# facebookresearch/robust_cvd

Hardware: NVIDIA H100
Metric: flow_residual_constraints_per_sec_per_gn_iteration (higher is better)
Workload: dtype f64

## Files before the change

### robust_cvd_b200/csrc/rcvd_api.cu

```cuda
#include <algorithm>
#include <chrono>
#include <cmath>
#include <cstdarg>
#include <cstdio>
#include <cstring>
#include <dlfcn.h>
#include <limits>
#include <string>
#include <vector>

#include <cub/device/device_segmented_sort.cuh>
#include "rcvd_eval.cuh"
#include "rcvd_linalg.cuh"
#include "rcvd_update.cuh"
#include "rcvd_plan.h"
#include "rcvd_host.h"

using namespace rcvd;

static thread_local std::string g_err = "";
int set_err(int code, const char* fmt, ...) {
  char buf[512]; va_list ap; va_start(ap, fmt); vsnprintf(buf, sizeof(buf), fmt, ap); va_end(ap);
  g_err = buf; return code;
}
// ... 293 lines not shown
    CK(cub::DeviceSegmentedSort::SortPairs(nullptr, tmp_bytes, d_k0, d_k1, d_i0, d_i1, (int)n, p->pairs.groups(), d_off, d_off + 1, p->stream));
    CK(cudaMallocAsync(&d_tmp, std::max<size_t>(tmp_bytes, 16), p->stream));
    CK(cub::DeviceSegmentedSort::SortPairs(d_tmp, tmp_bytes, d_k0, d_k1, d_i0, d_i1, (int)n, p->pairs.groups(), d_off, d_off + 1, p->stream));
    if ((rc = launch(p, k_gather_records, (unsigned)((n * 6 + 255) / 256), 256, 0, p->stream, false, p->pairs.dev.records, d_i1, n, d_sorted))) return rc;
    CK(cudaFreeAsync(d_tmp, p->stream));
    CK(cudaGetLastError());
    p->pairs.dev.records = d_sorted; p->records_sorted = true;
  }
  UP(p->d_in_range, frames_to_internal(uperm, p->in_range.data(), 1, 1, 1));
  UP(p->d_median, frames_to_internal(uperm, p->median.data(), 1, 1, 1));
  if (!p->adaptive.empty()) {
    const size_t G = p->adaptive.size() / N;
    UP(p->d_adaptive, frames_to_internal(uperm, p->adaptive.data(), G, G, G));
  }
  {
    std::vector<float> locs; const int gx = p->cfg.scale_grid_x, gy = p->cfg.scale_grid_y;
    for (int y = 0; y < gy; ++y) for (int x = 0; x < gx; ++x) {
      const float fx = -1.f + 2.f * x / (gx - 1);
      const float fy = -1.f + 2.f * y / (gy - 1);
      locs.push_back(fx); locs.push_back(fy);
    }
    p->nscale = (int)(locs.size() / 2);
    UP(p->d_scale_locs, locs);
  }
  p->first_frame = 0; p->last_frame = -1;
  { bool any = false; for (int f = 0; f < N; ++f) if (p->in_range[f]) { if (!any) { p->first_frame = f; any = true; } p->last_frame = f; } }
  p->part_reg = p->pairs.num_tiles;
  p->part_trip = p->part_reg + (reg_counts(p->cfg, L, N, p->nscale).total + 127) / 128;
  p->part_dp = p->part_trip + p->trips.num_tiles;
  p->npartial = p->part_dp + p->dpairs.num_tiles;
  return RCVD_OK;
}
#undef UP

static int allocate_storage(rcvd_problem* p) {
  const int N = p->N; const Layout& L = p->L; const int npad = L.npad, nLoff = p->plan.nLoff; const size_t bs = (size_t)npad * npad; int rc;
  const size_t Upad = (size_t)N * npad, U = (size_t)N * L.nf;
  DA(p->d_x, U); DA(p->d_xc, U); DA(p->d_xsave, U);
  DA(p->d_g, 2 * Upad + 8); p->d_diagH = p->d_g + Upad + 8;
  DA(p->d_S, Upad); DA(p->d_lmdiag, Upad); DA(p->d_D2, Upad); DA(p->d_gs, Upad); DA(p->d_rhs, Upad);
  DA(p->d_g2, Upad + 8); DA(p->d_delta, Upad);
  DA(p->d_ytmp, Upad); DA(p->d_y, Upad); DA(p->d_Sy, Upad); DA(p->d_Hy, Upad); DA(p->d_scal, SC_N); DA(p->d_active, Upad); DA(p->d_fail, 1);
  DA(p->d_potrf_progress, (size_t)N);
  DA(p->d_partial, (size_t)p->npartial);
  if (p->eval_only) { DA(p->d_H, 1); DA(p->d_Lb, 1); DA(p->d_T, 1); DA(p->d_invL, 1); DA(p->d_invT, 1); }
  else {
    DA(p->d_H, p->plan.hblocks.size() * bs); DA(p->d_Lb, (size_t)(N + nLoff) * bs); DA(p->d_T, (size_t)std::max(nLoff, 1) * bs);
    DA(p->d_invL, (size_t)N * bs); DA(p->d_invT, (size_t)N * npad * 16);
  }
#undef DA
  {
    bool encoded = false;
    typedef CUresult (*EncodeFn)(CUtensorMap*, CUtensorMapDataType, cuuint32_t, void*, const cuuint64_t*, const cuuint64_t*, const cuuint32_t*, const cuuint32_t*,
                                 CUtensorMapInterleave, CUtensorMapSwizzle, CUtensorMapL2promotion, CUtensorMapFloatOOBfill);
    void* fn = nullptr; cudaDriverEntryPointQueryResult qres;
    if (cudaGetDriverEntryPoint("cuTensorMapEncodeTiled", &fn, cudaEnableDefault, &qres) == cudaSuccess && fn && qres == cudaDriverEntryPointSuccess) {
      const cuuint64_t gdim[2] = {(cuuint64_t)npad, (cuuint64_t)std::max(nLoff, 1) * npad};
      const cuuint64_t gstr[1] = {(cuuint64_t)npad * sizeof(double)};
      const cuuint32_t box[2] = {16u, (cuuint32_t)p->plan.upd_rb};
      const cuuint32_t estr[2] = {1u, 1u};
      const CUresult r = ((EncodeFn)fn)(&p->tmapT, CU_TENSOR_MAP_DATA_TYPE_FLOAT64, 2, p->d_T, gdim, gstr, box, estr, CU_TENSOR_MAP_INTERLEAVE_NONE,
                                        CU_TENSOR_MAP_SWIZZLE_128B, CU_TENSOR_MAP_L2_PROMOTION_L2_128B, CU_TENSOR_MAP_FLOAT_OOB_FILL_NONE);
      encoded = (r == CUDA_SUCCESS);
    }
    cudaGetLastError();
    if (!encoded) return set_err(RCVD_ERR_CUDA, "cuTensorMapEncodeTiled unavailable or failed: the TMA update kernel cannot run");
    CK(cudaFuncSetAttribute(k_update_tma<1>, cudaFuncAttributeMaxDynamicSharedMemorySize, (int)upd_smem_bytes(p->plan.upd_rb, 1)));
    CK(cudaFuncSetAttribute(k_update_tma<2>, cudaFuncAttributeMaxDynamicSharedMemorySize, (int)upd_smem_bytes(p->plan.upd_rb, 2)));
  }
  CK(cudaMallocHost((void**)&p->h_scal, (SC_N + 2) * sizeof(double)));
  p->h_fail = (int*)(p->h_scal + SC_N);
  CK(cudaMemsetAsync(p->d_x, 0, U * sizeof(double), p->stream));
  CK(cudaMemsetAsync(p->d_lmdiag, 0, Upad * sizeof(double), p->stream));
  CK(cudaMemsetAsync(p->d_S, 0, Upad * sizeof(double), p->stream));
  CK(cudaMemsetAsync(p->d_active, 0, Upad, p->stream));
  if ((rc = enqueue_residuals<EvalMode::MarkActive>(p, p->d_x, nullptr))) return rc;
  if ((rc = launch(p, k_finalize_mask, (int)((Upad + 255) / 256), 256, 0, p->stream, false, p->cfg, L, p->d_active, N))) return rc;
  if (p->nranks > 1) {
    const int r = nccl::AllReduce(p->d_active, p->d_active, Upad, nccl::kUint8, nccl::kMax, p->comm, p->stream);
    if (r != 0) return set_err(RCVD_ERR_NCCL, "ncclAllReduce(active mask) failed");
  }
  FactorKernels& fk = p->fk = factor_kernels(npad);
  if (fk.trinv_bytes > kMaxDynSmem) return set_err(RCVD_ERR_INVALID, "frame block too large for the panel-inverse kernel (npad=%d)", npad);
  CK(cudaFuncSetAttribute(k_trinv, cudaFuncAttributeMaxDynamicSharedMemorySize, (int)fk.trinv_bytes));
  CK(cudaFuncSetAttribute(k_accumulate_fast, cudaFuncAttributeMaxDynamicSharedMemorySize, kFastSmem));
  CK(cudaFuncSetAttribute(k_accumulate_runs, cudaFuncAttributeMaxDynamicSharedMemorySize, kRunSmem));
  if (fk.trsm_ll) {
    CK(cudaFuncSetAttribute(k_trsm_ll<2>, cudaFuncAttributeMaxDynamicSharedMemorySize, (int)fk.trsm_ll2_bytes));
    CK(cudaFuncSetAttribute(k_trsm_ll<2, true>, cudaFuncAttributeMaxDynamicSharedMemorySize, (int)fk.trsm_ll2_bytes));
    CK(cudaOccupancyMaxActiveBlocksPerMultiprocessor(&fk.trsm2_ctas_per_sm, k_trsm_ll<2, true>, 128, fk.trsm_ll2_bytes));
  }
  if (fk.trsm_ll4) {
    CK(cudaFuncSetAttribute(k_trsm_ll<4>, cudaFuncAttributeMaxDynamicSharedMemorySize, (int)fk.trsm_ll4_bytes));
    CK(cudaFuncSetAttribute(k_trsm_ll<4, true>, cudaFuncAttributeMaxDynamicSharedMemorySize, (int)fk.trsm_ll4_bytes));
  }
  if (fk.potrf_smem) CK(cudaFuncSetAttribute(k_potrf_smem, cudaFuncAttributeMaxDynamicSharedMemorySize, (int)fk.potrf_bytes));
  return RCVD_OK;
}

static int build_structure(rcvd_problem* p) {
  if (p->nranks > 1 && !p->dpairs.frames.empty()) return set_err(RCVD_ERR_INVALID, "depth-normalisation pairs are not sharded: they need a single-GPU problem (nranks = 1)");
  free_all(p);
  CK(cudaSetDevice(p->device));
  std::vector<int32_t> graph = p->struct_pairs.empty() ? p->pairs.frames : p->struct_pairs;
  graph.insert(graph.end(), p->dpairs.frames.begin(), p->dpairs.frames.end());
  if (const char* e = make_factor_plan(p->plan, p->cfg, graph, p->trips.frames, p->order_slack, p->nranks, p->rank, p->dist_enabled, p->num_sms))
    return set_err(RCVD_ERR_INVALID, "%s", e);
  while (p->ev_side.size() < 2 * p->plan.levels.size()) { cudaEvent_t e; CK(cudaEventCreateWithFlags(&e, cudaEventDisableTiming)); p->ev_side.push_back(e); }
  int rc;
  if ((rc = upload_plan(p)) || (rc = set_up_problem_data(p)) || (rc = allocate_storage(p))) return rc;
  CK(cudaStreamSynchronize(p->stream));
  p->structure_ready = true;
  return RCVD_OK;
}

static int allreduce(rcvd_problem* p, double* buf, size_t count) {
  if (p->nranks <= 1) return RCVD_OK;
  const int r = nccl::AllReduce(buf, buf, count, nccl::kFloat64, nccl::kSum, p->comm, p->stream);
  if (r != 0) return set_err(RCVD_ERR_NCCL, "ncclAllReduce failed: %s", nccl::GetErrorString ? nccl::GetErrorString(r) : "?");
  return RCVD_OK;
}
struct Seg { size_t first, count; };
static int grouped(rcvd_problem* p, double* base, size_t unit, const std::vector<Seg>& segs, bool bcast) {
  int r = nccl::GroupStart();
  for (size_t i = 0; i < segs.size() && r == 0; ++i) {
    if (segs[i].count == 0) continue;
    const int root = (int)(i % (size_t)p->nranks);
    double* ptr = base + segs[i].first * unit;
    r = bcast ? nccl::Broadcast(ptr, ptr, segs[i].count * unit, nccl::kFloat64, root, p->comm, p->stream)
              : nccl::Reduce(ptr, ptr, segs[i].count * unit, nccl::kFloat64, nccl::kSum, root, p->comm, p->stream);
  }
  const int r2 = nccl::GroupEnd();
  if (r == 0) r = r2;
  if (r != 0) return set_err(RCVD_ERR_NCCL, "grouped NCCL %s failed: %s", bcast ? "broadcast" : "reduce", nccl::GetErrorString ? nccl::GetErrorString(r) : "?");
  return RCVD_OK;
}

struct FactorSolve {
  enum { P_LOAD = 0, P_POTRF, P_TRINV, P_TRSM, P_GEMM, P_SOLVE };
  rcvd_problem* p; const FactorPlan& pl; const FactorKernels& fk; const int N, npad, strips; cudaStream_t st, side, inv;
  int prof_level = 0;
  bool side_used = false, inv_used = false;
  int side_joined = -1;

  explicit FactorSolve(rcvd_problem* p_)
      : p(p_), pl(p_->plan), fk(p_->fk), N(p_->N), npad(p_->L.npad), strips((npad + kTrsmStrip - 1) / kTrsmStrip), st(p_->stream), side(p_->side_stream),
        inv(p_->inv_stream) {}

  void mark(int cls) {
    if (!p->prof) return;
    cudaEvent_t e; cudaEventCreate(&e); cudaEventRecord(e, st); p->prof->push_back({cls < 0 ? cls : (cls | (prof_level << 8)), e});
  }
  template <class... Params, class... Args>
  int launch(int path, void (*kernel)(Params...), dim3 grid, dim3 block, size_t smem, cudaStream_t s, bool pdl, Args... args) {
    if (int rc = ::launch(p, kernel, grid, block, smem, s, pdl, args...)) return rc;
    p->paths[path]++;
    return RCVD_OK;
  }
  int wait(cudaStream_t waiter, cudaStream_t from, cudaEvent_t e) {
    CK(cudaEventRecord(e, from)); CK(cudaStreamWaitEvent(waiter, e, 0));
    return RCVD_OK;
  }
  int join_all(int level) {
    if (side_used) { if (int rc = wait(st, side, p->ev_join)) return rc; side_joined = 2 * level - 1; }
    if (inv_used) { if (int rc = wait(st, inv, p->ev_inv_join)) return rc; inv_used = false; }
    return RCVD_OK;
  }

  bool trsm_deep(const Level& v) const { return strips * v.ntrsm <= p->num_sms && fk.trsm_ll4; }
  bool streamed(const Level& v) const {
    return fk.trsm_ll && v.nown > 0 && v.ntrsm > 0 && fk.potrf_smem && strips * v.ntrsm <= (trsm_deep(v) ? 1 : fk.trsm2_ctas_per_sm) * p->num_sms;
  }

  int factor_diagonal(const int* frames, int nfr, bool pdl) {
    if (fk.potrf_smem)
      return launch(LP_POTRF_SMEM, k_potrf_smem, dim3(nfr), dim3(kPotrfSmemThreads), fk.potrf_bytes, st, pdl, p->d_Lb, p->d_invT, frames, npad,
                    p->d_fail, p->d_potrf_progress);
    for (int jb = 0; jb < npad / 16; ++jb) {
      if (int rc = launch(LP_POTRF_PANEL, k_potrf_panel, dim3(nfr), dim3(kPotrfThreads), 0, st, false, p->d_Lb, p->d_invT, frames, npad, jb, p->d_fail)) return rc;
      const int m = npad - (jb + 1) * 16, n64 = (m + 63) / 64;
      if (m > 0) { if (int rc = launch(LP_OTHER, k_potrf_trail, dim3(n64 * (n64 + 1) / 2, nfr), dim3(128), 0, st, false, p->d_Lb, frames, npad, jb)) return rc; }
    }
    return RCVD_OK;
  }

  int trsm(const Level& lv, const int* frames, int nfr, bool chain) {
    const bool inv_stream = fk.trsm_ll && p->overlap;
    if (inv_stream) { if (int rc = wait(inv, st, p->ev_fork)) return rc; inv_used = true; }
    if (int rc = launch(LP_TRINV, k_trinv, dim3(npad / 16, nfr), dim3(256), fk.trinv_bytes, inv_stream ? inv : st, false,
                        p->d_Lb, p->d_invT, p->d_invL, frames, npad)) return rc;
    mark(P_TRINV);
    if (lv.ntrsm == 0) return RCVD_OK;
    int rc;
    if (fk.trsm_ll) {
      const bool deep = trsm_deep(lv);
      decltype(&k_trsm_ll<2>) kernel = deep ? (chain ? k_trsm_ll<4, true> : k_trsm_ll<4>) : (chain ? k_trsm_ll<2, true> : k_trsm_ll<2>);
      if (chain) p->paths[LP_TRSM_STREAMED]++;
      rc = launch(deep ? LP_TRSM_LL4 : LP_TRSM_LL2, kernel, dim3(strips, lv.ntrsm), dim3(128), deep ? fk.trsm_ll4_bytes : fk.trsm_ll2_bytes, st, chain,
                  p->d_T, p->d_Lb, p->d_invT, p->d_trsm_tasks + lv.trsm_off, npad, chain ? p->d_potrf_progress : nullptr);
    } else {
      const int tiles = (npad + 63) / 64;
      rc = launch(LP_TRSM_GEMM, k_gemm_nt, dim3(tiles, tiles, lv.ntrsm), dim3(128), 0, st, false, p->d_T, p->d_Lb, p->d_invL,
                  p->d_trsm_tasks + lv.trsm_off, npad);
    }
    if (rc) return rc;
    mark(P_TRSM);
    return RCVD_OK;
  }

  int update(cudaStream_t s, int off, int n) {
    if (n <= p->num_sms)
      return launch(LP_UPD_TMA2, k_update_tma<2>, dim3(n), dim3(UpdShape<2>::threads), upd_smem_bytes(pl.upd_rb, 2), s, false,
                    p->tmapT, p->d_Lb, p->d_upd_items + off, n, p->d_upd_pairs, npad, pl.upd_neff, pl.upd_rb, 0);
    int grid = std::min(n, 2 * p->num_sms);
    if (p->upd_ipc > 0) grid = std::max(grid, (n + p->upd_ipc - 1) / p->upd_ipc);
    if (grid < n) p->paths[LP_UPD_TMA1_MULTI]++;
    return launch(LP_UPD_TMA1, k_update_tma<1>, dim3(grid), dim3(UpdShape<1>::threads), upd_smem_bytes(pl.upd_rb, 1), s, false,
                  p->tmapT, p->d_Lb, p->d_upd_items + off, n, p->d_upd_pairs, npad, pl.upd_neff, pl.upd_rb, 0);
  }

  int updates(int li) {
    const Level& lv = pl.levels[li];
    const bool u2 = lv.nit2[0] + lv.nit2[1] > 0;
    const bool fork_late = li + 1 < (int)pl.levels.size() && streamed(pl.levels[li + 1]);
    if (p->overlap && u2 && !fork_late) { if (int rc = wait(side, st, p->ev_fork)) return rc; }
    if (p->overlap) {
      int s = -1;
      for (int q = side_joined + 1; q < 2 * li; ++q) { const Level& v = pl.levels[q / 2]; if (v.nit2[q % 2] > 0 && v.join[q % 2] <= li) s = q; }
      if (s >= 0) { CK(cudaStreamWaitEvent(st, p->ev_side[s], 0)); side_joined = s; }
    }
    if (lv.nit > 0) { if (int rc = update(st, lv.it_off, lv.nit)) return rc; mark(P_GEMM); }
    if (p->overlap && u2 && fork_late) { if (int rc = wait(side, st, p->ev_fork)) return rc; }
    for (int h = 0; h < 2; ++h) if (lv.nit2[h] > 0) {
      if (int rc = update(p->overlap ? side : st, lv.it2_off[h], lv.nit2[h])) return rc;
      mark(P_GEMM);
      if (p->overlap) { CK(cudaEventRecord(p->ev_side[2 * li + h], side)); side_used = true; }
    }
    return RCVD_OK;
  }

  int broadcast_level(int li) {
    std::vector<Seg> segs;
    for (int q = 0; q < p->nranks; ++q) segs.push_back({(size_t)pl.tseg[(li * p->nranks + q) * 2], (size_t)pl.tseg[(li * p->nranks + q) * 2 + 1]});
    return grouped(p, p->d_T, (size_t)npad * npad, segs, true);
  }
  int phase_boundary() {
    if (int rc = join_all(pl.LB)) return rc;
    const size_t bsz = (size_t)npad * npad;
    std::vector<Seg> invs, tr;
    for (int q = 0; q < p->nranks; ++q) invs.push_back({(size_t)pl.fa_off[q], (size_t)pl.fa_cnt[q]});
    for (int q = 0; q < p->nranks; ++q) tr.push_back({(size_t)pl.fb_off[q], (size_t)pl.fb_cnt[q]});
    for (int q = 0; q < p->nranks; ++q) tr.push_back({(size_t)N + (size_t)pl.bseg[2 * q], (size_t)pl.bseg[2 * q + 1]});
    if (int rc = grouped(p, p->d_invL, bsz, invs, true)) return rc;
    return grouped(p, p->d_Lb, bsz, tr, true);
  }

  int substitution() {
    CK(cudaMemcpyAsync(p->d_rhs, p->d_gs, (size_t)N * npad * sizeof(double), cudaMemcpyDeviceToDevice, st));
    const int LS = pl.sub_first_level;
    int rc;
    for (int l = 0; l < LS; ++l) {
      const Level& lv = pl.levels[l];
      if ((rc = launch(LP_SUB_LEVEL, k_fwd_diag, dim3((npad + 7) / 8, lv.nframes), dim3(256), 0, st, false, p->d_invL, p->d_rhs, p->d_ytmp,
                       p->d_lvl_frames + lv.frame_off, npad))) return rc;
      if (lv.nfwd > 0 && (rc = launch(LP_SUB_LEVEL, k_fwd_update, dim3((npad + 7) / 8, lv.nfwd), dim3(256), 0, st, false, p->d_T, p->d_ytmp, p->d_rhs,
                                      p->d_fwd_tasks + lv.fwd_off, npad))) return rc;
    }
    if (LS < (int)pl.levels.size() && !pl.sub_tasks.empty()) {
      CK(cudaMemsetAsync(p->d_sub_counters, 0, ((size_t)4 * N + 4) * sizeof(int), st));
      SubCounters cn; cn.ticket = p->d_sub_counters; cn.fin = p->d_sub_counters + 4; cn.fdone = cn.fin + N; cn.bin = cn.fdone + N; cn.bdone = cn.bin + N;
      cn.fin_need = p->d_sub_need; cn.bin_need = p->d_sub_need + N;
      const int ntasks = (int)pl.sub_tasks.size();
// ... 979 lines not shown
```

### robust_cvd_b200/csrc/rcvd_linalg.cuh

```cuda
#pragma once
#include "rcvd_device.cuh"
#include "rcvd_ptx.cuh"

namespace rcvd {

constexpr int kPotrfThreads = 256;

__global__ void __launch_bounds__(kPotrfThreads) k_potrf_panel(double* __restrict__ Lb, double* __restrict__ invT,
                                                                const int* __restrict__ frames, int npad, int jb, int* __restrict__ fail) {
  __shared__ double D[16][17];
  __shared__ double Di[16][17];
  const int frame = frames[blockIdx.x];
  double* A = Lb + (size_t)frame * npad * npad;
  double* iT = invT + (size_t)frame * npad * 16;
  const int tid = threadIdx.x;
  const int j0 = jb * 16;
  {
    const int r = tid >> 4, cc = tid & 15;
    D[r][cc] = (cc <= r) ? A[(size_t)(j0 + r) * npad + j0 + cc] : 0.0;
  }
  __syncthreads();
  if (tid < 32) {
    const int i = tid;
    for (int j = 0; j < 16; ++j) {
// ... 188 lines not shown
  POTRF_PHASE(1);
  for (int jb = 0; jb < nt; ++jb) {
    const double* D = tiles + (size_t)(jb * (jb + 1) / 2 + jb) * kTileSz;
    const double* pv = pinv + jb * 16;
    const int rows = (nt - jb - 1) * 16;
    int prow = -1;
    const int nwork = nw - 1, widx = warp - 1;
    if (warp == 0) { if (lane < 16 && rows > 0) prow = lane; } else if (widx * 32 + lane < rows - 16) prow = 16 + widx * 32 + lane;
    if (warp != 0) {
      if (jb > 0) publish(jb - 1);
      named_bar_sync<2, kPotrfSmemThreads>();
    }
    if (prow >= 0) {
      const int ti = jb + 1 + (prow >> 4), r = prow & 15;
      double* Tt = tiles + (size_t)(ti * (ti + 1) / 2 + jb) * kTileSz;
      double a[16];
#pragma unroll
      for (int q = 0; q < 16; q += 2) { const double2 v = *reinterpret_cast<const double2*>(&Tt[swz(r, q)]); a[q] = v.x; a[q + 1] = v.y; }
#pragma unroll
      for (int q = 0; q < 16; q += 2) {
        const double2 pq = *reinterpret_cast<const double2*>(&pv[q]);
        const double2 dq = *reinterpret_cast<const double2*>(&D[swz(q + 1, q)]);
        a[q] *= pq.x;
        a[q + 1] = (a[q + 1] - a[q] * dq.x) * pq.y;
#pragma unroll
        for (int c = 0; c < 16; ++c) if (c > q + 1) { const double2 l = *reinterpret_cast<const double2*>(&D[swz(c, q)]); a[c] -= a[q] * l.x; a[c] -= a[q + 1] * l.y; }
      }
#pragma unroll
      for (int q = 0; q < 16; q += 2) *reinterpret_cast<double2*>(&Tt[swz(r, q)]) = make_double2(a[q], a[q + 1]);
    } else if (warp == nw - 1 && lane < 16) {
      const int cidx = lane;
      double xcol[16];
#pragma unroll
      for (int r = 0; r < 16; ++r) xcol[r] = (r == cidx) ? 1.0 : 0.0;
#pragma unroll
      for (int q = 0; q < 16; q += 2) {
        const double2 pq = *reinterpret_cast<const double2*>(&pv[q]);
        const double2 dq = *reinterpret_cast<const double2*>(&D[swz(q + 1, q)]);
        xcol[q] *= pq.x;
        xcol[q + 1] = (xcol[q + 1] - xcol[q] * dq.x) * pq.y;
#pragma unroll
        for (int r = 0; r < 16; ++r) if (r > q + 1) { const double2 l = *reinterpret_cast<const double2*>(&D[swz(r, q)]); xcol[r] -= l.x * xcol[q]; xcol[r] -= l.y * xcol[q + 1]; }
      }
#pragma unroll
      for (int r = 0; r < 16; ++r) iT[(size_t)jb * 256 + r * 16 + cidx] = xcol[r];
    }
    POTRF_PHASE(2);
    if (warp != 0) named_bar_sync<3, kPotrfSmemThreads - 32>();
    POTRF_PHASE(3);
    const int m = nt - jb - 1, ntr = m * (m + 1) / 2;
    auto upd_tile = [&](int gi, int gj) -> double* {
      const double* Xi = tiles + (size_t)(gi * (gi + 1) / 2 + jb) * kTileSz;
      const double* Xj = tiles + (size_t)(gj * (gj + 1) / 2 + jb) * kTileSz;
      double* Ct = tiles + (size_t)(gi * (gi + 1) / 2 + gj) * kTileSz;
      double acc[2][2][2] = {{{0.0, 0.0}, {0.0, 0.0}}, {{0.0, 0.0}, {0.0, 0.0}}};
      tile_mma_nt(Xi, Xj, acc, g, t);
#pragma unroll
      for (int i = 0; i < 2; ++i)
#pragma unroll
        for (int j = 0; j < 2; ++j) {
          double2* ptr = reinterpret_cast<double2*>(&Ct[swz(i * 8 + g, j * 8 + 2 * t)]);
          double2 v = *ptr; v.x -= acc[i][j][0]; v.y -= acc[i][j][1]; *ptr = v;
        }
      return Ct;
    };
    if (warp == 0) {
      double* Ct = nullptr;
      if (ntr > 0) { __syncwarp(); Ct = upd_tile(jb + 1, jb + 1); }
      __threadfence_block();
      named_bar_arrive<2, kPotrfSmemThreads>();
      POTRF_PHASE(4);
      if (ntr > 0) { __syncwarp(); warp_chol16_blocked(Ct, pinv + (jb + 1) * 16, lane, fail); }
      POTRF_PHASE(5);
    } else {
      for (int tl = 1 + widx; tl < ntr; tl += nwork) { const int2 tij = tri_index(tl); upd_tile(jb + 1 + tij.x, jb + 1 + tij.y); }
    }
    POTRF_PHASE(6);
    __syncthreads();
    POTRF_PHASE(7);
  }
  if (warp != 0) publish(nt - 1);
}

__global__ void __launch_bounds__(256) k_trinv(const double* __restrict__ Lb, const double* __restrict__ invT, double* __restrict__ invL,
                                                const int* __restrict__ frames, int npad) {
  extern __shared__ double Z[];
  __shared__ double W[16][17];
  const int frame = frames[blockIdx.y];
  const int j = blockIdx.x;
  const int nt = npad / 16;
  double* Lrow_s = Z + (size_t)nt * 256;
  const int ldp = npad + 1;
  const double* A = Lb + (size_t)frame * npad * npad;
  const double* iT = invT + (size_t)frame * npad * 16;
  double* out = invL + (size_t)frame * npad * npad;
  const int tid = threadIdx.x, r = tid >> 4, c = tid & 15;
  for (int i = 0; i < j; ++i) out[(size_t)(i * 16 + r) * npad + j * 16 + c] = 0.0;
  Z[(size_t)j * 256 + tid] = iT[(size_t)j * 256 + tid];
  out[(size_t)(j * 16 + r) * npad + j * 16 + c] = Z[(size_t)j * 256 + tid];
  __syncthreads();
  for (int i = j + 1; i < nt; ++i) {
    const int kw = (i - j) * 16;
    for (int e = tid; e < 16 * kw; e += 256) { const int rr = e / kw, kk = e % kw; Lrow_s[rr * ldp + kk] = A[(size_t)(i * 16 + rr) * npad + j * 16 + kk]; }
    __syncthreads();
    double s0 = 0.0, s1 = 0.0, s2 = 0.0, s3 = 0.0;
    const double* lr = Lrow_s + r * ldp;
    const double* zp = Z + (size_t)j * 256 + c;
    for (int kk = 0; kk < kw; kk += 4) {
      s0 += lr[kk] * zp[(size_t)kk * 16]; s1 += lr[kk + 1] * zp[(size_t)(kk + 1) * 16];
      s2 += lr[kk + 2] * zp[(size_t)(kk + 2) * 16]; s3 += lr[kk + 3] * zp[(size_t)(kk + 3) * 16];
    }
    W[r][c] = (s0 + s1) + (s2 + s3);
    __syncthreads();
    double zv = 0.0;
    const double* ti = iT + (size_t)i * 256;
#pragma unroll
    for (int q = 0; q < 16; ++q) zv -= ti[r * 16 + q] * W[q][c];
    Z[(size_t)i * 256 + tid] = zv;
    out[(size_t)(i * 16 + r) * npad + j * 16 + c] = zv;
    __syncthreads();
  }
}

struct TrsmTask { int dst; int src; int kframe; };

constexpr int kGemmLd = 20;

template <int NI, int NJ>
__device__ __forceinline__ void gemm_stage(const double* __restrict__ as, const double* __restrict__ bsm, double (&acc)[4][4][2], int wm, int wn, int g, int t) {
#pragma unroll
  for (int k4 = 0; k4 < 4; ++k4) {
    double af[NI > 0 ? NI : 1], bf[NJ > 0 ? NJ : 1];
#pragma unroll
    for (int i = 0; i < NI; ++i) af[i] = as[(wm + i * 8 + g) * kGemmLd + k4 * 4 + t];
#pragma unroll
    for (int j = 0; j < NJ; ++j) bf[j] = bsm[(wn + j * 8 + g) * kGemmLd + k4 * 4 + t];
#pragma unroll
    for (int i = 0; i < NI; ++i)
#pragma unroll
      for (int j = 0; j < NJ; ++j) dmma_8x8x4(acc[i][j][0], acc[i][j][1], af[i], bf[j]);
  }
}

__global__ void __launch_bounds__(128, 4) k_gemm_nt(double* __restrict__ T, const double* __restrict__ Lb, const double* __restrict__ invL,
                                                  const TrsmTask* __restrict__ tasks, int npad) {
  __shared__ __align__(16) double As[2][64 * kGemmLd];
  __shared__ __align__(16) double Bs[2][64 * kGemmLd];
  const TrsmTask task = tasks[blockIdx.z];
  const int m0 = blockIdx.y * 64, n0 = blockIdx.x * 64;
  const size_t bs = (size_t)npad * npad;
  const int tid = threadIdx.x, warp = tid >> 5, lane = tid & 31;
  const int wm = (warp >> 1) * 32, wn = (warp & 1) * 32;
  const int g = lane >> 2, t = lane & 3;
  const int kchunks = min(npad, n0 + 64) / 16;
  const int ni = min(4, max(0, (npad - (m0 + wm)) / 8)), nj = min(4, max(0, (npad - (n0 + wn)) / 8));
  double acc[4][4][2];
#pragma unroll
  for (int i = 0; i < 4; ++i)
#pragma unroll
    for (int j = 0; j < 4; ++j) { acc[i][j][0] = 0.0; acc[i][j][1] = 0.0; }

  auto load_stage = [&](int st, int kk) {
    const double* Ag = Lb + (size_t)task.src * bs + kk * 16;
    const double* Bg = invL + (size_t)task.kframe * bs + kk * 16;
#pragma unroll
    for (int q = 0; q < 4; ++q) {
      const int cidx = tid + q * 128;
      const int row = cidx >> 3, kc = (cidx & 7) * 2;
      const bool va = (m0 + row) < npad, vb = (n0 + row) < npad;
      cp_async16(&As[st][row * kGemmLd + kc], Ag + (size_t)(va ? m0 + row : 0) * npad + kc, va);
      cp_async16(&Bs[st][row * kGemmLd + kc], Bg + (size_t)(vb ? n0 + row : 0) * npad + kc, vb);
    }
    cp_async_commit();
  };

  load_stage(0, 0);
  for (int kk = 0; kk < kchunks; ++kk) {
    const int st = kk & 1;
    if (kk + 1 < kchunks) { load_stage(st ^ 1, kk + 1); cp_async_wait<1>(); } else { cp_async_wait<0>(); }
    __syncthreads();
    const double* as = As[st]; const double* bsm = Bs[st];
    if (ni == 4 && nj == 4) gemm_stage<4, 4>(as, bsm, acc, wm, wn, g, t);
    else if (ni == 4 && nj == 2) gemm_stage<4, 2>(as, bsm, acc, wm, wn, g, t);
    else if (ni == 2 && nj == 4) gemm_stage<2, 4>(as, bsm, acc, wm, wn, g, t);
    else if (ni == 2 && nj == 2) gemm_stage<2, 2>(as, bsm, acc, wm, wn, g, t);
    __syncthreads();
  }
  double* C = T + (size_t)task.dst * bs;
#pragma unroll
  for (int i = 0; i < 4; ++i) {
    const int row = m0 + wm + i * 8 + g;
    if (row >= npad) continue;
#pragma unroll
    for (int j = 0; j < 4; ++j) {
      const int col = n0 + wn + j * 8 + 2 * t;
      if (col >= npad) continue;
      *reinterpret_cast<double2*>(C + (size_t)row * npad + col) = make_double2(acc[i][j][0], acc[i][j][1]);
    }
  }
}

__global__ void __launch_bounds__(128, 4) k_potrf_trail(double* __restrict__ Lb, const int* __restrict__ frames, int npad, int jb) {
  __shared__ __align__(16) double Ps[2][64 * kGemmLd];
  const int frame = frames[blockIdx.y];
  double* A = Lb + (size_t)frame * npad * npad;
  const int j0 = jb * 16, j1 = j0 + 16;
// ... 92 lines not shown
        __syncthreads();
        ready = s_ready;
      }
      for (; staged < min(ready, jt + kTrsmAhead); ++staged) stage(staged);
      cp_async_wait_upto3(staged - 1 - jt);
    } else {
      cp_async_wait<kTrsmAhead - 1>();
    }
    __syncthreads();
    const double* ls = Ls + (size_t)(jt % kTrsmAhead) * 16 * ld; const double* dsm = Ds + (jt % kTrsmAhead) * 320;
    double acc[NI][2][2];
#pragma unroll
    for (int i = 0; i < NI; ++i) { acc[i][0][0] = acc[i][0][1] = acc[i][1][0] = acc[i][1][1] = 0.0; }
    {
      double af[2][4][NI], bf[2][4][2];
      auto frag = [&](int kt, int buf) {
#pragma unroll
        for (int q = 0; q < 4; ++q) {
#pragma unroll
          for (int i = 0; i < NI; ++i) af[buf][q][i] = Xs[(size_t)(wr + i * 8 + g) * ld + kt * 16 + q * 4 + t];
#pragma unroll
          for (int j = 0; j < 2; ++j) bf[buf][q][j] = ls[(size_t)(j * 8 + g) * ld + kt * 16 + q * 4 + t];
        }
      };
      if (jt > 0) frag(0, 0);
      for (int kt = 0; kt < jt; kt += 2) {
        if (kt + 1 < jt) frag(kt + 1, 1);
#pragma unroll
        for (int q = 0; q < 4; ++q)
#pragma unroll
          for (int i = 0; i < NI; ++i)
#pragma unroll
            for (int j = 0; j < 2; ++j) dmma_8x8x4(acc[i][j][0], acc[i][j][1], af[0][q][i], bf[0][q][j]);
        if (kt + 1 < jt) {
          if (kt + 2 < jt) frag(kt + 2, 0);
#pragma unroll
          for (int q = 0; q < 4; ++q)
#pragma unroll
            for (int i = 0; i < NI; ++i)
#pragma unroll
              for (int j = 0; j < 2; ++j) dmma_8x8x4(acc[i][j][0], acc[i][j][1], af[1][q][i], bf[1][q][j]);
        }
      }
    }
#pragma unroll
    for (int i = 0; i < NI; ++i)
#pragma unroll
      for (int j = 0; j < 2; ++j) {
        double2* ptr = reinterpret_cast<double2*>(&Xs[(size_t)(wr + i * 8 + g) * ld + jt * 16 + j * 8 + 2 * t]);
        double2 v = *ptr; v.x -= acc[i][j][0]; v.y -= acc[i][j][1]; *ptr = v;
      }
    __syncwarp();
    double out[NI][2][2];
#pragma unroll
    for (int i = 0; i < NI; ++i) { out[i][0][0] = out[i][0][1] = out[i][1][0] = out[i][1][1] = 0.0; }
#pragma unroll
    for (int k4 = 0; k4 < 4; ++k4) {
      double af[NI], bf[2];
#pragma unroll
      for (int i = 0; i < NI; ++i) af[i] = Xs[(size_t)(wr + i * 8 + g) * ld + jt * 16 + k4 * 4 + t];
#pragma unroll
      for (int j = 0; j < 2; ++j) bf[j] = dsm[(j * 8 + g) * 20 + k4 * 4 + t];
#pragma unroll
      for (int i = 0; i < NI; ++i)
#pragma unroll
        for (int j = 0; j < 2; ++j) dmma_8x8x4(out[i][j][0], out[i][j][1], af[i], bf[j]);
    }
    __syncwarp();
#pragma unroll
    for (int i = 0; i < NI; ++i)
#pragma unroll
      for (int j = 0; j < 2; ++j) {
        const int r = wr + i * 8 + g, cidx = jt * 16 + j * 8 + 2 * t;
        const double2 v = make_double2(out[i][j][0], out[i][j][1]);
        *reinterpret_cast<double2*>(&Xs[(size_t)r * ld + cidx]) = v;
        if (r < rows) *reinterpret_cast<double2*>(&X[(size_t)(m0 + r) * npad + cidx]) = v;
      }
    __syncthreads();
    if constexpr (!kStreamed) stage(jt + kTrsmAhead);
  }
  if constexpr (kStreamed) griddep_wait();
}


__global__ void __launch_bounds__(256) k_fwd_diag(const double* __restrict__ invL, const double* __restrict__ rhs, double* __restrict__ y,
                                                   const int* __restrict__ frames, int npad) {
  const int frame = frames[blockIdx.y];
  const int row = blockIdx.x * 8 + (threadIdx.x >> 5);
  const int lane = threadIdx.x & 31;
  if (row >= npad) return;
  const double* M = invL + (size_t)frame * npad * npad + (size_t)row * npad;
  const double* b = rhs + (size_t)frame * npad;
  double s = 0.0;
  for (int q = lane; q <= row; q += 32) s += M[q] * b[q];
  s = warp_sum(s);
  if (lane == 0) y[(size_t)frame * npad + row] = s;
}
struct SolveTask { int blk; int r; int k; };
__global__ void __launch_bounds__(256) k_fwd_update(const double* __restrict__ T, const double* __restrict__ y, double* __restrict__ rhs,
                                                     const SolveTask* __restrict__ tasks, int npad) {
  const SolveTask tk = tasks[blockIdx.y];
  const int row = blockIdx.x * 8 + (threadIdx.x >> 5);
  const int lane = threadIdx.x & 31;
  if (row >= npad) return;
  const double* M = T + (size_t)tk.blk * npad * npad + (size_t)row * npad;
  const double* v = y + (size_t)tk.k * npad;
  double s = 0.0;
  for (int q = lane; q < npad; q += 32) s += M[q] * v[q];
  s = warp_sum(s);
  if (lane == 0) red_add(rhs + (size_t)tk.r * npad + row, -s);
}
__global__ void __launch_bounds__(256) k_bwd_update(const double* __restrict__ T, const double* __restrict__ x, double* __restrict__ y,
                                                     const SolveTask* __restrict__ tasks, int npad) {
  __shared__ double red[8][33];
  const SolveTask tk = tasks[blockIdx.y];
  const int cl = threadIdx.x & 31, rg = threadIdx.x >> 5;
  const int j = blockIdx.x * 32 + cl;
  double acc = 0.0;
  if (j < npad) {
    const double* M = T + (size_t)tk.blk * npad * npad + j;
    const double* xr = x + (size_t)tk.r * npad;
    for (int i = rg; i < npad; i += 8) acc += M[(size_t)i * npad] * xr[i];
  }
  red[rg][cl] = acc;
  __syncthreads();
  if (rg == 0 && j < npad) {
    double s = 0.0;
#pragma unroll
    for (int q = 0; q < 8; ++q) s += red[q][cl];
    if (s != 0.0) red_add(y + (size_t)tk.k * npad + j, -s);
  }
}
__global__ void __launch_bounds__(256) k_bwd_diag(const double* __restrict__ invL, const double* __restrict__ y, double* __restrict__ x,
                                                   const int* __restrict__ frames, int npad) {
  __shared__ double red[8][33];
  const int frame = frames[blockIdx.y];
  const int cl = threadIdx.x & 31, rg = threadIdx.x >> 5;
  const int j = blockIdx.x * 32 + cl;
  double acc = 0.0;
  if (j < npad) {
    const double* M = invL + (size_t)frame * npad * npad + j;
    const double* v = y + (size_t)frame * npad;
    const int i0 = j - (j % 8) + rg;
    for (int i = (i0 < j ? i0 + 8 : i0); i < npad; i += 8) acc += M[(size_t)i * npad] * v[i];
  }
  red[rg][cl] = acc;
  __syncthreads();
  if (rg == 0 && j < npad) {
    double s = 0.0;
#pragma unroll
    for (int q = 0; q < 8; ++q) s += red[q][cl];
    x[(size_t)frame * npad + j] = s;
  }
}

constexpr int kSubChunk = 64;
constexpr int kSubThreads = 256;
struct SubTask { int type; int blk; int r; int k; int chunk; };
struct SubCounters { int* ticket; int* fin; int* fdone; int* bin; int* bdone; const int* fin_need; const int* bin_need; };

__device__ __forceinline__ void sub_wait(const int* c, int need) { while (ld_acquire_gpu(c) < need) __nanosleep(20); }

__device__ __forceinline__ double2 ldcg2(const double* p) { return __ldcg(reinterpret_cast<const double2*>(p)); }

__global__ void __launch_bounds__(kSubThreads) k_substitution(const double* __restrict__ invL, const double* __restrict__ T, double* rhs, double* y, double* x,
                                                              const SubTask* __restrict__ tasks, int ntasks, SubCounters cn, int npad) {
// ... 10 lines not shown
    const SubTask tk = tasks[ti];
    const int c0 = tk.chunk * kSubChunk, c1 = min(npad, c0 + kSubChunk);
    const double* vin = tk.type == 0 ? rhs + (size_t)tk.k * npad : (tk.type == 2 ? x + (size_t)tk.r * npad : y + (size_t)tk.k * npad);
    const double* M = (tk.type == 0 || tk.type == 3) ? invL + (size_t)tk.k * bs : T + (size_t)tk.blk * bs;
    auto dep_wait = [&]() {
      if (tid == 0) {
        if (tk.type == 0) sub_wait(cn.fin + tk.k, cn.fin_need[tk.k]);
        else if (tk.type == 1) sub_wait(cn.fdone + tk.k, nchunks);
        else if (tk.type == 2) sub_wait(cn.bdone + tk.r, nchunks);
        else { sub_wait(cn.fdone + tk.k, nchunks); sub_wait(cn.bin + tk.k, cn.bin_need[tk.k]); }
      }
      __syncthreads();
    };
    if (tk.type <= 1) {
      constexpr int RW = kSubChunk / (kSubThreads / 32);
      const int r0 = c0 + warp * RW;
      double acc[RW];
#pragma unroll
      for (int i = 0; i < RW; ++i) acc[i] = 0.0;
      for (int qb = 0; qb < npad; qb += 256) {
        double2 m[4][RW];
#pragma unroll
        for (int qi = 0; qi < 4; ++qi) {
          const int q = qb + qi * 64 + 2 * lane;
#pragma unroll
          for (int i = 0; i < RW; ++i) {
            const int row = r0 + i;
            const int len = tk.type == 0 ? row + 1 : npad;
            m[qi][i] = (row < c1 && q < len) ? *reinterpret_cast<const double2*>(M + (size_t)row * npad + q) : make_double2(0.0, 0.0);
            if (q + 1 >= len) m[qi][i].y = 0.0;
          }
        }
        if (qb == 0) dep_wait();
        double2 v[4];
#pragma unroll
        for (int qi = 0; qi < 4; ++qi) { const int q = qb + qi * 64 + 2 * lane; v[qi] = q < npad ? ldcg2(vin + q) : make_double2(0.0, 0.0); }
#pragma unroll
        for (int qi = 0; qi < 4; ++qi)
#pragma unroll
          for (int i = 0; i < RW; ++i) acc[i] += m[qi][i].x * v[qi].x + m[qi][i].y * v[qi].y;
      }
#pragma unroll
      for (int i = 0; i < RW; ++i) {
        const double sum = warp_sum(acc[i]);
        const int row = r0 + i;
        if (lane == 0 && row < c1) { if (tk.type == 0) y[(size_t)tk.k * npad + row] = sum; else red_add(rhs + (size_t)tk.r * npad + row, -sum); }
      }
    } else {
      const int cl = tid & 31, rg = tid >> 5, j = c0 + 2 * cl;
      double ax = 0.0, ay = 0.0;
      const int ifirst = tk.type == 3 ? j + ((rg - j) & 7) : rg;
      for (int ib = ifirst; ib < npad || ib == ifirst; ib += 256) {
        double2 m[32];
#pragma unroll
        for (int u = 0; u < 32; ++u) { const int i = ib + 8 * u; m[u] = (i < npad && j < c1) ? *reinterpret_cast<const double2*>(M + (size_t)i * npad + j) : make_double2(0.0, 0.0); }
        if (ib == ifirst) dep_wait();
        double vi[32];
#pragma unroll
        for (int u = 0; u < 32; ++u) { const int i = ib + 8 * u; vi[u] = i < npad ? __ldcg(vin + i) : 0.0; }
#pragma unroll
        for (int u = 0; u < 32; ++u) { const int i = ib + 8 * u; ax += m[u].x * vi[u]; if (tk.type != 3 || i > j) ay += m[u].y * vi[u]; }
      }
      red[rg * (kSubChunk + 2) + 2 * cl] = ax; red[rg * (kSubChunk + 2) + 2 * cl + 1] = ay;
      __syncthreads();
      if (tid < kSubChunk && c0 + tid < c1) {
        double sum = 0.0;
#pragma unroll
        for (int q = 0; q < 8; ++q) sum += red[q * (kSubChunk + 2) + tid];
        if (tk.type == 3) x[(size_t)tk.k * npad + c0 + tid] = sum; else red_add(y + (size_t)tk.k * npad + c0 + tid, -sum);
      }
    }
    __syncthreads();
    if (tid == 0) red_release_add(tk.type == 0 ? cn.fdone + tk.k : (tk.type == 1 ? cn.fin + tk.r : (tk.type == 2 ? cn.bin + tk.k : cn.bdone + tk.k)), 1);
  }
}

struct FactorKernels {
  bool potrf_smem, trsm_ll, trsm_ll4;
  size_t potrf_bytes, trsm_ll2_bytes, trsm_ll4_bytes, trinv_bytes, substitution_bytes;
  int trsm2_ctas_per_sm;
};
inline FactorKernels factor_kernels(int npad) {
  const size_t potrf = potrf_smem_bytes(npad), ll2 = trsm_ll_smem_bytes(npad, 2), ll4 = trsm_ll_smem_bytes(npad, 4);
  const size_t trinv = (size_t)(npad * 16 + 16 * (npad + 1)) * sizeof(double);
  const size_t sub = (size_t)8 * (kSubChunk + 2) * sizeof(double);
  return {potrf <= kMaxDynSmem, ll2 <= kMaxDynSmem, ll4 <= kMaxDynSmem, potrf, ll2, ll4, trinv, sub, 0};
}

struct HBlock { int lblk; int r; int c; };
__global__ void __launch_bounds__(256) k_load_factor(const double* __restrict__ H, double* __restrict__ Lb, const HBlock* __restrict__ lb,
                                                      const double* __restrict__ S, const double* __restrict__ D2, int npad, int nf, int neff,
                                                      const int* __restrict__ blist, int nload, int nfill) {
  const size_t bs = (size_t)npad * npad;
  if ((int)blockIdx.y >= nload) {
    const int ph = npad - neff, per = ph * (npad + neff);
    const long q = ((long)(blockIdx.y - nload) * gridDim.x + blockIdx.x) * 256 + threadIdx.x;
    if (per == 0 || q >= (long)nfill * per) return;
    const int f = (int)(q / per), e = (int)(q % per), r = e - ph * npad;
    const int i = r < 0 ? neff + e / npad : r / ph, j = r < 0 ? e % npad : neff + r % ph;
    Lb[(size_t)blist[nload + f] * bs + (size_t)i * npad + j] = 0.0;
    return;
  }
  const int bid = blist[blockIdx.y];
  const HBlock b = lb[bid];
  const int e = blockIdx.x * 256 + threadIdx.x;
  if (e >= npad * npad) return;
  const int i = e / npad, j = e % npad;
  double v = 0.0;
  if (b.r == b.c) {
    if (j > i) v = 0.0;
    else if (i >= nf) v = (i == j) ? 1.0 : 0.0;
    else {
      v = H[(size_t)b.lblk * bs + e] * S[(size_t)b.r * npad + i] * S[(size_t)b.c * npad + j];
      if (i == j) v += D2[(size_t)b.r * npad + i];
    }
  } else if (i < nf && j < nf) {
    v = H[(size_t)b.lblk * bs + e] * S[(size_t)b.r * npad + i] * S[(size_t)b.c * npad + j];
  }
  Lb[(size_t)bid * bs + e] = v;
}
__host__ __device__ inline int load_factor_pad_rows(int npad, int neff, int nfill) {
  const long per = (long)(npad - neff) * (npad + neff), row = (long)((npad * npad + 255) / 256) * 256;
  return (int)(((long)nfill * per + row - 1) / row);
}

__global__ void __launch_bounds__(256) k_spmv_sym(const double* __restrict__ H, const HBlock* __restrict__ hb, const double* __restrict__ v,
                                                   double* __restrict__ out, int npad, const int* __restrict__ blist) {
  const int bid = blist ? blist[blockIdx.y] : blockIdx.y;
  const HBlock b = hb[bid];
  const int row = blockIdx.x * 8 + (threadIdx.x >> 5);
  const int lane = threadIdx.x & 31;
  if (row >= npad) return;
  const double* M = H + (size_t)bid * npad * npad + (size_t)row * npad;
  const double* vc = v + (size_t)b.c * npad;
  const double vr = v[(size_t)b.r * npad + row];
  double s = 0.0;
  if (b.r == b.c) {
    for (int q = lane; q <= row; q += 32) {
      const double m = M[q];
      s += m * vc[q];
      if (q < row && m != 0.0) red_add(out + (size_t)b.c * npad + q, m * vr);
    }
  } else {
    for (int q = lane; q < npad; q += 32) {
      const double m = M[q];
      s += m * vc[q];
      if (m != 0.0 && vr != 0.0) red_add(out + (size_t)b.c * npad + q, m * vr);
    }
  }
  s = warp_sum(s);
  if (lane == 0 && s != 0.0) red_add(out + (size_t)b.r * npad + row, s);
}

}
```

Before: 84.82 million.

## Rewrite triangular inverse kernel as strip-based DMMA solve with cp.async staging

Replaces the per-column-block scalar triangular inverse with a strip-parallel kernel that computes inverse rows using FP64 tensor-core MMA (dmma_16x8x4). L panels and diagonal inverses are staged into shared memory with cp.async double-buffering when shared memory permits, and the kernel falls back to direct global loads otherwise. The aim is to cut the scalar FMA and sync-heavy cost of the inverse step in the factorization. In exchange it changes the grid/block shape, writes the output transposed (column-wise stores), and adds more complex synchronization.

After: 86.56 million (median of 6 runs). 1.02x the previous value.

```diff
diff --git a/robust_cvd_b200/csrc/rcvd_api.cu b/robust_cvd_b200/csrc/rcvd_api.cu
--- a/robust_cvd_b200/csrc/rcvd_api.cu
+++ b/robust_cvd_b200/csrc/rcvd_api.cu
@@ -399,7 +399,7 @@
   }
   FactorKernels& fk = p->fk = factor_kernels(npad);
   if (fk.trinv_bytes > kMaxDynSmem) return set_err(RCVD_ERR_INVALID, "frame block too large for the panel-inverse kernel (npad=%d)", npad);
-  CK(cudaFuncSetAttribute(k_trinv, cudaFuncAttributeMaxDynamicSharedMemorySize, (int)fk.trinv_bytes));
+  CK(cudaFuncSetAttribute(fk.trsm_ll ? k_trinv<true> : k_trinv<false>, cudaFuncAttributeMaxDynamicSharedMemorySize, (int)fk.trinv_bytes));
   CK(cudaFuncSetAttribute(k_accumulate_fast, cudaFuncAttributeMaxDynamicSharedMemorySize, kFastSmem));
   CK(cudaFuncSetAttribute(k_accumulate_runs, cudaFuncAttributeMaxDynamicSharedMemorySize, kRunSmem));
   if (fk.trsm_ll) {
@@ -504,7 +504,7 @@
   int trsm(const Level& lv, const int* frames, int nfr, bool chain) {
     const bool inv_stream = fk.trsm_ll && p->overlap;
     if (inv_stream) { if (int rc = wait(inv, st, p->ev_fork)) return rc; inv_used = true; }
-    if (int rc = launch(LP_TRINV, k_trinv, dim3(npad / 16, nfr), dim3(256), fk.trinv_bytes, inv_stream ? inv : st, false,
+    if (int rc = launch(LP_TRINV, fk.trsm_ll ? k_trinv<true> : k_trinv<false>, dim3(strips, nfr), dim3(128), fk.trinv_bytes, inv_stream ? inv : st, false,
                         p->d_Lb, p->d_invT, p->d_invL, frames, npad)) return rc;
     mark(P_TRINV);
     if (lv.ntrsm == 0) return RCVD_OK;
diff --git a/robust_cvd_b200/csrc/rcvd_linalg.cuh b/robust_cvd_b200/csrc/rcvd_linalg.cuh
--- a/robust_cvd_b200/csrc/rcvd_linalg.cuh
+++ b/robust_cvd_b200/csrc/rcvd_linalg.cuh
@@ -294,46 +294,6 @@
   if (warp != 0) publish(nt - 1);
 }
 
-__global__ void __launch_bounds__(256) k_trinv(const double* __restrict__ Lb, const double* __restrict__ invT, double* __restrict__ invL,
-                                                const int* __restrict__ frames, int npad) {
-  extern __shared__ double Z[];
-  __shared__ double W[16][17];
-  const int frame = frames[blockIdx.y];
-  const int j = blockIdx.x;
-  const int nt = npad / 16;
-  double* Lrow_s = Z + (size_t)nt * 256;
-  const int ldp = npad + 1;
-  const double* A = Lb + (size_t)frame * npad * npad;
-  const double* iT = invT + (size_t)frame * npad * 16;
-  double* out = invL + (size_t)frame * npad * npad;
-  const int tid = threadIdx.x, r = tid >> 4, c = tid & 15;
-  for (int i = 0; i < j; ++i) out[(size_t)(i * 16 + r) * npad + j * 16 + c] = 0.0;
-  Z[(size_t)j * 256 + tid] = iT[(size_t)j * 256 + tid];
-  out[(size_t)(j * 16 + r) * npad + j * 16 + c] = Z[(size_t)j * 256 + tid];
-  __syncthreads();
-  for (int i = j + 1; i < nt; ++i) {
-    const int kw = (i - j) * 16;
-    for (int e = tid; e < 16 * kw; e += 256) { const int rr = e / kw, kk = e % kw; Lrow_s[rr * ldp + kk] = A[(size_t)(i * 16 + rr) * npad + j * 16 + kk]; }
-    __syncthreads();
-    double s0 = 0.0, s1 = 0.0, s2 = 0.0, s3 = 0.0;
-    const double* lr = Lrow_s + r * ldp;
-    const double* zp = Z + (size_t)j * 256 + c;
-    for (int kk = 0; kk < kw; kk += 4) {
-      s0 += lr[kk] * zp[(size_t)kk * 16]; s1 += lr[kk + 1] * zp[(size_t)(kk + 1) * 16];
-      s2 += lr[kk + 2] * zp[(size_t)(kk + 2) * 16]; s3 += lr[kk + 3] * zp[(size_t)(kk + 3) * 16];
-    }
-    W[r][c] = (s0 + s1) + (s2 + s3);
-    __syncthreads();
-    double zv = 0.0;
-    const double* ti = iT + (size_t)i * 256;
-#pragma unroll
-    for (int q = 0; q < 16; ++q) zv -= ti[r * 16 + q] * W[q][c];
-    Z[(size_t)i * 256 + tid] = zv;
-    out[(size_t)(i * 16 + r) * npad + j * 16 + c] = zv;
-    __syncthreads();
-  }
-}
-
 struct TrsmTask { int dst; int src; int kframe; };
 
 constexpr int kGemmLd = 20;
@@ -592,6 +552,103 @@
   if constexpr (kStreamed) griddep_wait();
 }
 
+constexpr int kTrinvAhead = 2;
+__host__ __device__ inline size_t trinv_smem_bytes(int npad, bool staged) {
+  return staged ? trsm_ll_smem_bytes(npad, kTrinvAhead) : (size_t)kTrsmStrip * (npad + 4) * sizeof(double);
+}
+
+template <bool kStaged>
+__global__ void __launch_bounds__(128) k_trinv(const double* __restrict__ Lb, const double* __restrict__ invT, double* __restrict__ invL,
+                                                const int* __restrict__ frames, int npad) {
+  extern __shared__ __align__(16) double Ys[];
+  const int ld = npad + 4;
+  double* Ls = Ys + (size_t)kTrsmStrip * ld;
+  double* Ds = Ls + (size_t)kTrinvAhead * 16 * ld;
+  const int frame = frames[blockIdx.y];
+  const int m0 = blockIdx.x * kTrsmStrip, j0 = 2 * blockIdx.x;
+  const double* Lk = Lb + (size_t)frame * npad * npad;
+  const double* iT = invT + (size_t)frame * npad * 16;
+  double* out = invL + (size_t)frame * npad * npad;
+  const int tid = threadIdx.x, warp = tid >> 5, lane = tid & 31, g = lane >> 2, t = lane & 3;
+  const int nt = npad / 16;
+  auto stage = [&](int jt) {
+    if (jt < nt) {
+      double* ls = Ls + (size_t)(jt % kTrinvAhead) * 16 * ld; double* dsm = Ds + (jt % kTrinvAhead) * 320;
+      const int r = tid >> 3, c0 = (tid & 7) * 2;
+      const double* src = Lk + (size_t)(jt * 16 + r) * npad;
+      for (int c = m0 + c0; c < jt * 16; c += 16) cp_async16(&ls[(size_t)r * ld + c], src + c);
+      cp_async16(&dsm[r * 20 + c0], iT + (size_t)jt * 256 + r * 16 + c0);
+    }
+    cp_async_commit();
+  };
+  if constexpr (kStaged) {
+#pragma unroll
+    for (int q = 0; q < kTrinvAhead; ++q) stage(j0 + q);
+  }
+  for (int c = tid >> 4; c < m0; c += 8) {
+    const int q = m0 + (tid & 15) * 2;
+    if (q < npad) *reinterpret_cast<double2*>(&out[(size_t)c * npad + q]) = make_double2(0.0, 0.0);
+  }
+  const int wr = (warp >> 1) * 16, wc = (warp & 1) * 8;
+  auto pair_sync = [&]() { if (warp < 2) named_bar_sync<1, 64>(); else named_bar_sync<2, 64>(); };
+  const double* ya = Ys + (size_t)(wr + g) * ld + t;
+  for (int jt = j0; jt < nt; ++jt) {
+    if constexpr (kStaged) {
+      cp_async_wait<kTrinvAhead - 1>();
+      __syncthreads();
+    }
+    const double* lrow = kStaged ? Ls + (size_t)((jt % kTrinvAhead) * 16 + wc + g) * ld + t : Lk + (size_t)(jt * 16 + wc + g) * npad + t;
+    double di[4];
+#pragma unroll
+    for (int k4 = 0; k4 < 4; ++k4)
+      di[k4] = kStaged ? Ds[(jt % kTrinvAhead) * 320 + (wc + g) * 20 + k4 * 4 + t] : __ldg(&iT[(size_t)jt * 256 + (wc + g) * 16 + k4 * 4 + t]);
+    double acc[2][4] = {{0.0, 0.0, 0.0, 0.0}, {0.0, 0.0, 0.0, 0.0}};
+    {
+      double af[2][4][2], bf[2][4];
+      auto frag = [&](int kt, int buf) {
+#pragma unroll
+        for (int q = 0; q < 4; ++q) {
+          bf[buf][q] = kStaged ? lrow[kt * 16 + q * 4] : __ldg(&lrow[kt * 16 + q * 4]);
+          af[buf][q][0] = ya[kt * 16 + q * 4];
+          af[buf][q][1] = ya[(size_t)8 * ld + kt * 16 + q * 4];
+        }
+      };
+      if (jt > j0) frag(j0, 0);
+      for (int kt = j0; kt < jt; kt += 2) {
+        if (kt + 1 < jt) frag(kt + 1, 1);
+#pragma unroll
+        for (int q = 0; q < 4; ++q) dmma_16x8x4(acc[0][0], acc[0][1], acc[0][2], acc[0][3], af[0][q][0], af[0][q][1], bf[0][q]);
+        if (kt + 1 < jt) {
+          if (kt + 2 < jt) frag(kt + 2, 0);
+#pragma unroll
+          for (int q = 0; q < 4; ++q) dmma_16x8x4(acc[1][0], acc[1][1], acc[1][2], acc[1][3], af[1][q][0], af[1][q][1], bf[1][q]);
+        }
+      }
+    }
+    const int cg = jt * 16 + wc + 2 * t;
+#pragma unroll
+    for (int i = 0; i < 2; ++i) {
+      const int rg = m0 + wr + i * 8 + g;
+      const double tx = (rg == cg ? 1.0 : 0.0) - (acc[0][2 * i] + acc[1][2 * i]);
+      const double ty = (rg == cg + 1 ? 1.0 : 0.0) - (acc[0][2 * i + 1] + acc[1][2 * i + 1]);
+      *reinterpret_cast<double2*>(&Ys[(size_t)(wr + i * 8 + g) * ld + cg]) = make_double2(tx, ty);
+    }
+    pair_sync();
+    double y[4] = {0.0, 0.0, 0.0, 0.0};
+#pragma unroll
+    for (int k4 = 0; k4 < 4; ++k4) dmma_16x8x4(y[0], y[1], y[2], y[3], ya[jt * 16 + k4 * 4], ya[(size_t)8 * ld + jt * 16 + k4 * 4], di[k4]);
+    if constexpr (kStaged) { __syncthreads(); stage(jt + kTrinvAhead); } else { pair_sync(); }
+#pragma unroll
+    for (int i = 0; i < 2; ++i) {
+      const int r = wr + i * 8 + g, rg = m0 + r;
+      const double vx = rg > cg ? 0.0 : y[2 * i], vy = rg > cg + 1 ? 0.0 : y[2 * i + 1];
+      *reinterpret_cast<double2*>(&Ys[(size_t)r * ld + cg]) = make_double2(vx, vy);
+      if (rg < npad) { out[(size_t)cg * npad + rg] = vx; out[(size_t)(cg + 1) * npad + rg] = vy; }
+    }
+    if constexpr (!kStaged) pair_sync();
+  }
+}
+
 
 __global__ void __launch_bounds__(256) k_fwd_diag(const double* __restrict__ invL, const double* __restrict__ rhs, double* __restrict__ y,
                                                    const int* __restrict__ frames, int npad) {
@@ -768,7 +825,7 @@
 };
 inline FactorKernels factor_kernels(int npad) {
   const size_t potrf = potrf_smem_bytes(npad), ll2 = trsm_ll_smem_bytes(npad, 2), ll4 = trsm_ll_smem_bytes(npad, 4);
-  const size_t trinv = (size_t)(npad * 16 + 16 * (npad + 1)) * sizeof(double);
+  const size_t trinv = trinv_smem_bytes(npad, ll2 <= kMaxDynSmem);
   const size_t sub = (size_t)8 * (kSubChunk + 2) * sizeof(double);
   return {potrf <= kMaxDynSmem, ll2 <= kMaxDynSmem, ll4 <= kMaxDynSmem, potrf, ll2, ll4, trinv, sub, 0};
 }
```
